# medical-genomics-group/ci-gwas

Measured on AMD Instinct MI355X. Metric: ci_tests_per_sec, higher is better.
Workload: dtype f32; 1 GPU; cusk level sweep, one LD block 10000 SNPs x 20 traits, N=16384, alpha=0.0001, max level 5 (north_star headline); correlation matrix from synthetic .bed (Kendall-npn/Pearson) resident in HBM; n_variables=10020, engine=cusk

## Files before the change

ci-gwas_amd/csrc/cusk_internal.h:

```cpp
#pragma once
#include <hip/hip_runtime.h>

#include <cstdint>
#include <cstdio>
#include <string>
#include <vector>

#include "../../include/cusk_hip.h"

namespace cusk {

constexpr int kML = CUSK_ML;
constexpr int kLevels = CUSK_ML + 2;
constexpr unsigned long long kNone = ~0ull;
constexpr int kNumClasses = 5;
constexpr int kClassCap[kNumClasses] = {39, 63, 127, 191, 1 << 30};
constexpr int kThreads = 256;
constexpr int kTmajMinLevelDefault = 6;
constexpr int kCounterSlots = 512;
constexpr size_t kLdsLimit = 160 * 1024;

struct DevBuf
{
    void *p = nullptr;
    size_t cap = 0;
    hipError_t ensure(size_t bytes)
    {
        if (bytes <= cap) return hipSuccess;
        if (p) (void)hipFree(p);
        p = nullptr;
        cap = 0;
        size_t want = bytes + bytes / 4 + 256;
        hipError_t e = hipMalloc(&p, want);
        if (e == hipSuccess) cap = want;
        return e;
    }
    void release()
    {
        if (p) (void)hipFree(p);
        p = nullptr;
        cap = 0;
    }
    template <typename T>
    T *as() const
    {
        return reinterpret_cast<T *>(p);
    }
};

struct LevelCounters;
struct HostGate;
// ... 40 lines not shown
    void *res_pinned = nullptr;
    size_t res_pinned_cap = 0;
    cusk::DevBuf rv, rpos, sel, wpre;
    long long nrec = 0;
    cusk::LevelCounters *hcnt = nullptr;
    unsigned long long *hslots = nullptr;
    long long *hrec_base = nullptr;
    unsigned long long *hcanon = nullptr;
    int *hflag = nullptr;
    std::vector<unsigned long long> binom_host;
    long long binom_rows = 0;
    cusk::HostGate *hgate = nullptr, *hgate_dev = nullptr;
    int run_seq = 0;
    long long item_cap_cur = 0;
    hipEvent_t ev_main[2] = {nullptr, nullptr};
    hipEvent_t ev_run[2] = {nullptr, nullptr};
    hipEvent_t ev_k0[cusk::kLevels], ev_k1[cusk::kLevels], ev_l0[cusk::kLevels], ev_l1[cusk::kLevels];

    int opt_fast = 1;
    int opt_validate = 0;
    int opt_corr_fp4 = 1;
    int opt_pair = 1;
    int opt_rows = 1;
    int opt_vec = 1;
    int opt_overlap = 1;
    int opt_corr_popcount = 0;
    int opt_corr_mxp_f32 = 0;
    int opt_assume_symmetric = 0;
    long long opt_queue_cap = 4ll << 20;
    int opt_hostprof = 0;
    int opt_tmaj_validate_stride = 1;
    int opt_max_staged_classes = -1;
    int opt_tmaj_min_level = cusk::kTmajMinLevelDefault;
    long long opt_chunk = 2048;
    long long opt_chunk0 = 512;
    long long opt_chunk0_low = 256;
    int opt_vec_threads = 64;
    long long opt_item_cap = 1ll << 20;
    int opt_lookahead = 2;
    int opt_sync2 = 1;
    int opt_l1_threads = 0;
    int opt_l1_lds_row = 1;
    int opt_timing = 1;
    long long opt_sep_ws_budget = 4ll << 30;

    int shard_rank = 0, shard_world = 1;
    int shard_host_staging = 0;
    cusk_exchange_fn shard_fn = nullptr;
    void *shard_user = nullptr;
    void *shard_host = nullptr;
    size_t shard_host_cap = 0;

    cusk::DevBuf bed_dev, phen_dev, mean_dev, std_dev, planes, mxp_dev, pxp_dev, mxp_bq;
    cusk::DevBuf pc_masks, pc_counts;
    cusk::DevBuf corr_tab[2];
    void *corr_tab_pinned[2] = {nullptr, nullptr};
    size_t corr_tab_pinned_cap[2] = {0, 0};
    hipEvent_t ev_corr[5] = {nullptr, nullptr, nullptr, nullptr, nullptr};
    float corr_ms[4] = {0, 0, 0, 0};
};

namespace cusk {

inline int fail(cusk_engine *e, int code, const std::string &msg)
{
    if (e) e->err = msg;
// ... 35 lines not shown
```

ci-gwas_amd/csrc/engine.hip:

```cpp
#include <algorithm>
#include <atomic>
#include <chrono>
#include <cmath>
#include <cstdlib>
#include <cstring>

#include "sweep_common.h"

namespace cusk {

static unsigned long long binom_sat(int n, int k)
{
    if (k < 0 || k > n) return 0;
    if (k > n - k) k = n - k;
    unsigned long long r = 1;
    const unsigned long long cap = 1ull << 62;
    for (int i = 1; i <= k; i++)
    {
        unsigned long long f = (unsigned long long)(n - k + i);
        if (r > cap / f) return cap;
        r = r * f / (unsigned long long)i;
    }
    return r;
}
// ... 22 lines not shown
    const float *C;
    const float *Ness;
    float ess_uniform;
    const int *Ginit;
    const float *Th;
    const int *time_index;
    int n;
    int maxlevel;
    const int2 *row_range = nullptr;
    int max_span = 0;
    long long level0_pairs = 0;
};

constexpr size_t kCtlCnt = 0;
constexpr size_t kCtlSlots = (kCtlCnt + sizeof(LevelCounters) * kLevels + 15) & ~(size_t)15;
constexpr size_t kCtlRecBase = (kCtlSlots + sizeof(unsigned long long) * kLevels * kCounterSlots * 4 + 15) & ~(size_t)15;
constexpr size_t kCtlCanon = (kCtlRecBase + sizeof(long long) * (kLevels + 1) + 15) & ~(size_t)15;
constexpr size_t kCtlSym = (kCtlCanon + sizeof(unsigned long long) * kLevels * kCounterSlots + 15) & ~(size_t)15;
constexpr size_t kCtlBytes = kCtlSym + 16;

struct LevelPlan
{
    SweepParams sp;
    FinalizeParams fp;
    long long nitems[kNumClasses];
    bool use_pair = false, use_fast = false, use_rows = false, filter_ok = true;
    size_t pair_lds = 0;
    bool redone = false;
    bool known_items = false;
    int maxdeg_bound = 0;
    int staged_classes = 0;
    unsigned long long chunk0 = 0;
    bool tmaj = false;
    bool force_exact = false;
};

static int run_levels(cusk_engine *e, const RunArgs &a, cusk_stats *st)
{
    const int n = a.n;
    if (n <= 0 || a.C == nullptr || a.Th == nullptr) return fail(e, CUSK_ERR_ARG, "bad arguments");
    const auto hp_t0 = std::chrono::steady_clock::now();
    std::string hp_log;
    auto hp_mark = [&](const char *what) {
        if (!e->opt_hostprof) return;
        const double us = std::chrono::duration<double, std::micro>(std::chrono::steady_clock::now() - hp_t0).count();
        char buf[64];
        std::snprintf(buf, sizeof(buf), " %s=%.1f", what, us);
        hp_log += buf;
    };
    CUSK_HIP(e, hipSetDevice(e->device));
    hipStream_t s = e->stream;
    const int words = (n + 63) / 64;
    e->n = n;
    e->words = words;
    e->mode = a.mode;
    e->have_result = false;
    e->nrec = 0;
    cusk_stats local;
    std::memset(&local, 0, sizeof(local));
    const bool het = (a.Ness != nullptr);
    const bool het0 = het && a.mode == 0;
    const int last_level = std::min(kML, a.maxlevel);
    const bool sharded = e->shard_world > 1;
    if (sharded && !e->shard_fn) return fail(e, CUSK_ERR_ARG, "row sharding needs an exchange function");

    const size_t bm = sizeof(unsigned long long) * (size_t)n * words;
// ... 101 lines not shown
        }
        const bool fork = (nonempty > 1) && (e->opt_overlap != 0);
        if (fork)
        {
            CUSK_HIP(e, hipEventRecord(e->ev_fork, s));
            CUSK_HIP(e, hipStreamWaitEvent(e->stream2, e->ev_fork, 0));
        }
        bool first = true;
        for (int c = 0; c < kNumClasses; c++)
        {
            if (!may[c]) continue;
            hipStream_t cs = (fork && !first) ? e->stream2 : s;
            first = false;
            sp.items = e->items[l & 1][c].as<int2>();
            sp.cap = kClassCap[c];
            sp.cls = c;
            sp.chunk = (c == 0) ? pl.chunk0 : chunk;
            sp.item_cap = item_cap;
            sp.grid_cap = item_cap;
            if (l >= 2 && !pl.use_pair && !pl.tmaj)
            {
                const int dmax = std::min(pl.maxdeg_bound, kClassCap[c]);
                const unsigned long long sets = binom_sat(dmax, l);
                const unsigned long long per_row = sets / sp.chunk + 1ull;
                if (per_row < (1ull << 40)) sp.grid_cap = std::min<long long>(item_cap, (long long)(per_row * (unsigned long long)n));
            }
            sp.validate = e->opt_validate ? std::max(1, e->opt_tmaj_validate_stride) : 0;
            if (pl.use_pair && !exact_only)
                CUSK_HIP(e, launch_pair(a.mode, sp, pl.pair_lds, cs));
            else if (pl.tmaj && pl.use_fast && !exact_only)
                CUSK_HIP(e, launch_sweep_tmaj(a.mode, l, sp, c, cs));
            else if (pl.use_fast && !exact_only && !het && e->opt_vec && !e->opt_validate && c < kNumClasses - 1 &&
                     sweep_vec_lds_bytes(c) <= kLdsLimit && l < kVecMaxLevel)
                CUSK_HIP(e, launch_sweep_vec(a.mode, l, sp, c, c == 0 ? e->opt_vec_threads : kThreads, cs));
            else if (pl.use_fast && !exact_only)
                CUSK_HIP(e, launch_sweep_fast(a.mode, het, l, e->opt_validate != 0, sp, c, cs));
            else
                CUSK_HIP(e, launch_sweep_exact(a.mode, het, l, sp, c, cs));
        }
        if (fork)
        {
            CUSK_HIP(e, hipEventRecord(e->ev_join, e->stream2));
            CUSK_HIP(e, hipStreamWaitEvent(s, e->ev_join, 0));
        }
        if (pl.use_fast && !exact_only) CUSK_HIP(e, launch_recheck(a.mode, het, l, sp, s));
        return CUSK_OK;
    };
    auto launch_level_finalize = [&](int l) -> int {
        if (a.mode != 0) return CUSK_OK;
        LevelPlan &pl = plan[l];
        pl.fp.qcap = qcap_gate[l];
        CUSK_HIP(e, launch_finalize(l, pl.fp, s));
        return CUSK_OK;
    };

    auto shard_join = [&](int l) -> int {
        LevelPlan &pl = plan[l];
        if (pl.use_fast && l >= 2)
        {
            CUSK_HIP(e, hipMemcpyAsync(e->hcnt + l, dcnt + l, sizeof(LevelCounters), hipMemcpyDeviceToHost, s));
            CUSK_HIP(e, hipStreamSynchronize(s));
            if (e->hcnt[l].qcount > (unsigned long long)e->opt_queue_cap)
            {
                pl.redone = true;
                local.exact_fallbacks++;
                qcap_gate[l] = ~0ull;
                const int rc = launch_level_sweeps(l, true);
// ... 92 lines not shown
                    if (rc != CUSK_OK) return rc;
                    if (!e->hgate[k].active) break;
                }
            }
            if (e->opt_timing == 2) CUSK_HIP(e, hipEventRecord(e->ev_l0[l], s));
            LevelPlan &pl = plan[l];
            pl.redone = false;
            pl.known_items = false;
            const bool first_build = (l == 1 && first_pass);
            int *off_l = (l == 1) ? e->off1.as<int>() : e->off[cs].as<int>();
            PlanArgs pa;
            pa.deg = e->deg.as<int>();
            pa.off = off_l;
            for (int c = 0; c < kNumClasses; c++) pa.items[c] = e->items[cs][c].as<int2>();
            pa.n = n;
            pa.L = l;
            pa.binom = e->binom.as<unsigned long long>();
            pa.chunk = chunk;
            {
                float th_l;
                if (het)
                    th_l = a.Th[0];
                else if (a.mode == 0)
                    th_l = a.Th[l];
                else
                    th_l = uniform_ess_threshold(a.Th[0], a.ess_uniform, l);
                const bool vec0 = (e->opt_fast != 0) && l >= 2 && l < kVecMaxLevel && th_l >= kThMinFilter && !het && e->opt_vec &&
                                  !e->opt_validate && staged_classes > 0;
                const unsigned long long c0 = (l <= 4) ? (unsigned long long)std::max<long long>(e->opt_chunk0_low, 64) : chunk0;
                plan[l].chunk0 = vec0 ? c0 : chunk;
                plan[l].tmaj = (e->opt_fast != 0) && !plan[l].force_exact && l >= std::max(2, e->opt_tmaj_min_level) && l <= kML &&
                               th_l >= kThMinFilter && !het && symmetric && !sharded;
                if (plan[l].tmaj) plan[l].chunk0 = chunk;
            }
            pa.chunk0 = plan[l].chunk0;
            pa.Lsets = plan[l].tmaj ? l + 1 : l;
            pa.staged_classes = staged_classes;
            pa.pair_mode = ((l == 1) && !first_build && plan[l].use_pair && !plan[l].use_rows) ? 1 : 0;
            pa.cnt = dcnt + l;
            pa.prev = (l >= 2) ? dcnt + (l - 1) : nullptr;
            pa.prev_qcap = (l >= 2) ? qcap_gate[l - 1] : ~0ull;
            pa.item_cap = item_cap;
            pa.shard_rank = e->shard_rank;
            pa.shard_world = e->shard_world;
            pa.gate = e->hgate_dev + l;
            pa.seq = run_seq;
            pa.sym = (l == 1 && !e->opt_assume_symmetric && !a.row_range) ? dsym : nullptr;
            pa.blocks = e->planblk.as<unsigned long long>();
            pa.blk_seq = ++e->plan_seq;
            if (first_build && e->binom_rows <= 0)
            {
                CUSK_HIP(e, e->binom.ensure(sizeof(unsigned long long) * kBinomStride));
                pa.binom = e->binom.as<unsigned long long>();
            }
            CUSK_HIP(e, launch_plan(pa, s));
            planned_last = l;
            if (first_build)
            {
                hp_mark("plan1_enq");
                int *const rec_l_before = (a.mode == 0) ? e->rec_l.as<int>() : nullptr;
                const size_t rec_l_cleared = rec_l_before ? e->rec_l.cap : 0;
                if (rec_l_cleared) CUSK_HIP(e, hipMemsetAsync(rec_l_before, 0, rec_l_cleared, s));
                int rc = wait_gate(1);
                if (rc != CUSK_OK) return rc;
                hp_mark("gate1");
                symmetric = (e->hgate[1].sym == 0) || (e->opt_assume_symmetric != 0) || (a.row_range != nullptr);
// ... 71 lines not shown
                maxdeg2 = e->hgate[2].maxdeg;
            }
            {
                pl.maxdeg_bound = maxdeg1;
                if (maxdeg2 >= 0 && l >= 2) pl.maxdeg_bound = std::min(pl.maxdeg_bound, maxdeg2);
                const int k = l - 1 - lookahead;
                if (k >= 1 && e->hgate[k].seq == run_seq && e->hgate[k].active) pl.maxdeg_bound = std::min(pl.maxdeg_bound, e->hgate[k].maxdeg);
                pl.staged_classes = staged_classes;
            }

            SweepParams &sp = pl.sp;
            sp.C = a.C;
            sp.Ness = a.Ness;
            sp.n = n;
            sp.level = l;
            sp.off = off_l;
            sp.nbr = e->nbr[cs].as<int>();
            sp.best = e->best[cs].as<unsigned long long>();
            sp.adj = e->adj.as<unsigned long long>();
            sp.deg = e->deg.as<int>();
            sp.words = words;
            sp.items = nullptr;
            sp.binom = e->binom.as<unsigned long long>();
            sp.time_index = e->ti.as<int>();
            sp.has_ti = (a.mode == 1 && a.time_index != nullptr) ? 1 : 0;
            sp.chunk = chunk;
            sp.cap = 0;
            sp.cls = 0;
            sp.item_cap = item_cap;
            sp.grid_cap = item_cap;
            sp.cnt = dcnt + l;
            sp.row_range = a.row_range;
            sp.max_span = a.row_range ? a.max_span : n;
            sp.slots = dslots + (size_t)l * kCounterSlots * 4;
            if (het)
                sp.th = a.Th[0];
            else if (a.mode == 0)
                sp.th = a.Th[l];
            else
                sp.th = uniform_ess_threshold(a.Th[0], a.ess_uniform, l);
            {
                const double tq = std::tanh((double)sp.th);
                sp.t2 = (float)(tq * tq);
                pl.filter_ok = (sp.th >= kThMinFilter);
                if (!pl.filter_ok) pl.use_fast = false;
            }
            sp.queue = nullptr;
            sp.qcap = 0;
            qcap_gate[l] = ~0ull;
            if (pl.use_fast)
            {
                sp.queue = e->queue.as<RecheckEntry>();
                sp.qcap = (unsigned long long)e->opt_queue_cap;
                qcap_gate[l] = sp.qcap;
            }
            FinalizeParams &fp = pl.fp;
            fp.C = a.C;
            fp.n = n;
            fp.off = sp.off;
            fp.nbr = sp.nbr;
            fp.best = sp.best;
            fp.sel = pl.use_rows ? e->sel.as<unsigned>() : nullptr;
            fp.level = l;
            fp.adj = sp.adj;
            fp.deg = sp.deg;
            fp.words = words;
// ... 274 lines not shown
{
    if (!e || !key) return CUSK_ERR_ARG;
    const std::string k(key);
    if (k == "fast")
        e->opt_fast = (int)value;
    else if (k == "validate")
        e->opt_validate = (int)value;
    else if (k == "corr_fp4")
        e->opt_corr_fp4 = (int)value;
    else if (k == "pair")
        e->opt_pair = (int)value;
    else if (k == "rows")
        e->opt_rows = (int)value;
    else if (k == "vec")
        e->opt_vec = (int)value;
    else if (k == "overlap")
        e->opt_overlap = (int)value;
    else if (k == "corr_popcount")
        e->opt_corr_popcount = (int)value;
    else if (k == "corr_mxp_f32")
        e->opt_corr_mxp_f32 = (int)value;
    else if (k == "assume_symmetric")
        e->opt_assume_symmetric = (int)value;
    else if (k == "queue_capacity" && value > 0)
        e->opt_queue_cap = value;
    else if (k == "chunk" && value >= 256)
        e->opt_chunk = value;
    else if (k == "max_staged_classes")
        e->opt_max_staged_classes = (int)value;
    else if (k == "tmaj_validate_stride" && value >= 1 && (value & (value - 1)) == 0)
        e->opt_tmaj_validate_stride = (int)value;
    else if (k == "tmaj_min_level")
        e->opt_tmaj_min_level = (int)value;
    else if (k == "hostprof")
        e->opt_hostprof = (int)value;
    else if (k == "chunk0_low" && value >= 64)
        e->opt_chunk0_low = value;
    else if (k == "chunk0" && value >= 64)
        e->opt_chunk0 = value;
    else if (k == "vec_threads" && (value == 64 || value == 128 || value == 256))
        e->opt_vec_threads = (int)value;
    else if (k == "item_capacity" && value > 0)
    {
        e->opt_item_cap = value;
        e->item_cap_cur = 0;
    }
    else if (k == "lookahead" && value >= 0)
        e->opt_lookahead = (int)value;
    else if (k == "timing")
        e->opt_timing = (int)value;
    else if (k == "l1_threads" && (value == 0 || value == 256 || value == 512))
        e->opt_l1_threads = (int)value;
    else if (k == "l1_lds_row" && (value == 0 || value == 1))
        e->opt_l1_lds_row = (int)value;
    else if (k == "sync2")
        e->opt_sync2 = (int)value;
    else if (k == "sepselect_ws_bytes" && value > 0)
        e->opt_sep_ws_budget = value;
    else
        return fail(e, CUSK_ERR_ARG, "unknown option " + k);
    return CUSK_OK;
}

extern "C" int cusk_engine_set_row_shard(cusk_engine *e, int rank, int world, cusk_exchange_fn fn, void *user, int host_staging)
{
    if (!e) return CUSK_ERR_ARG;
// ... 514 lines not shown
```

ci-gwas_amd/csrc/sweep_common.h:

```cpp
#pragma once
#include "cusk_internal.h"

namespace cusk {

constexpr int kBinomStride = 16;
constexpr int kVecMaxLevel = 9;
constexpr float kThMinFilter = 2e-3f;

struct RowInfo
{
    int cls;
    int base;
    int nchunks;
    int pad;
};

struct RecheckEntry
{
    int x;
    int k2;
    unsigned long long rank;
};

struct LevelCounters
// ... 19 lines not shown
    long long class_items[kNumClasses];
};

struct SweepParams
{
    const float *C;
    const float *Ness;
    int n;
    int level;
    const int *off;
    const int *nbr;
    unsigned long long *best;
    unsigned long long *adj;
    int *deg;
    int words;
    const int2 *items;
    const unsigned long long *binom;
    const int *time_index;
    int has_ti;
    float th;
    float t2;
    unsigned long long chunk;
    int cap;
    int cls;
    long long item_cap;
    long long grid_cap;
    LevelCounters *cnt;
    unsigned long long *slots;
    RecheckEntry *queue;
    unsigned long long qcap;
    int validate;
    const int2 *row_range;
    int max_span;
};

struct FinalizeParams
{
    const float *C;
    int n;
    const int *off;
    const int *nbr;
    const unsigned long long *best;
    const unsigned *sel;
    int level;
    unsigned long long *adj;
    int *deg;
    int words;
    const unsigned long long *binom;
    const int *off1;
    const int *wpre1;
    const unsigned long long *adj0;
    int *rec_x, *rec_y, *rec_l, *rec_s;
    long long rec_cap;
    const int4 *meta;
    const LevelCounters *cnt;
    unsigned long long qcap;
    unsigned long long *slots;
    unsigned long long *canon;
};

__host__ __device__ inline size_t align16(size_t x) { return (x + 15) & ~(size_t)15; }

struct LdsLayout
{
    size_t nbr, best, ti, sub, ess, total;
};
// ... 82 lines not shown
}

__device__ __forceinline__ bool clear_edge(unsigned long long *adj, int *deg, int words, int X, int Y)
{
    const unsigned long long o1 = atomicAnd(&adj[(size_t)X * words + (Y >> 6)], ~(1ull << (Y & 63)));
    const unsigned long long o2 = atomicAnd(&adj[(size_t)Y * words + (X >> 6)], ~(1ull << (X & 63)));
    const bool f1 = (o1 >> (Y & 63)) & 1ull, f2 = (o2 >> (X & 63)) & 1ull;
    if (f1) atomicSub(&deg[X], 1);
    if (f2) atomicSub(&deg[Y], 1);
    return f1;
}
#endif

hipError_t launch_sweep_exact(int mode, bool het, int L, const SweepParams &p, int cls, hipStream_t st);
hipError_t launch_recheck(int mode, bool het, int L, const SweepParams &p, hipStream_t st);
hipError_t launch_finalize(int L, const FinalizeParams &p, hipStream_t st);
hipError_t launch_record_z(int L, const float *C, int n, const int *x, const int *y, const int *l, const int *s, long long stride,
                           long long count, float *z, hipStream_t st);
constexpr int kRecBlock = 1024;
hipError_t launch_rec_count(const int *rec_l, long long slots, int *counts, hipStream_t st);
hipError_t launch_rec_compact(const int *rec_l, const int *rec_x, const int *rec_y, const int *rec_s, long long rec_cap,
                              long long slots, const long long *block_off, int *out_x, int *out_y, int *out_l, int *out_s,
                              long long out_stride, hipStream_t st);
hipError_t launch_sweep_fast(int mode, bool het, int L, bool validate, const SweepParams &p, int cls, hipStream_t st);
hipError_t launch_sweep_tmaj(int mode, int L, const SweepParams &p, int cls, hipStream_t st);
__host__ __device__ inline int tmaj_prefixes_per_lane(int d, int s, unsigned long long chunk)
{
    const unsigned long long r = (unsigned long long)(d - 1 - s);
    const unsigned long long pairs = r * (r - 1ull) / 2ull;
    const unsigned long long k = chunk / ((unsigned long long)kThreads * (pairs ? pairs : 1ull));
    return (int)(k < 1ull ? 1ull : (k > 64ull ? 64ull : k));
}
hipError_t launch_sweep_vec(int mode, int L, const SweepParams &p, int cls, int threads, hipStream_t st);
unsigned persistent_grid(const void *kernel, int threads, size_t lds);
size_t sweep_vec_lds_bytes(int cls);
hipError_t launch_level0(const float *C, const float *Ness, const int *Ginit, unsigned long long *adj, int n, int words,
                         float th, int *asym_flag, hipStream_t st);
hipError_t launch_level0_batch(const float *C, const float *Ness, unsigned long long *adj, unsigned long long *adj0, int *deg, int n,
                               int words, const int2 *row_range, float th, hipStream_t st);
hipError_t launch_degree(const unsigned long long *adj, int *deg, int n, int words, unsigned long long *adj0, hipStream_t st);
hipError_t launch_fill_nbr(const unsigned long long *adj, const int *off, int *nbr, unsigned long long *best, int n, int words,
                           int *wpre, const LevelCounters *cnt, const int2 *row_range, hipStream_t st);
struct PlanArgs
{
    const int *deg;
    int *off;
    int2 *items[kNumClasses];
    int n, L;
    int Lsets;
    const unsigned long long *binom;
    unsigned long long chunk, chunk0;
    int staged_classes, pair_mode;
    LevelCounters *cnt;
    const LevelCounters *prev;
    unsigned long long prev_qcap;
    long long item_cap;
    int shard_rank, shard_world;
    HostGate *gate;
    int seq;
    const int *sym;
    unsigned long long *blocks;
    unsigned blk_seq;
};
hipError_t launch_plan(const PlanArgs &a, hipStream_t st);
hipError_t launch_expand_records(const int *rec_s, const int *rec_l, long long rec_cap, long long count, int *out,
                                 hipStream_t st);
// ... 18 lines not shown
```

ci-gwas_amd/csrc/sweep_vec.hip:

```cpp
#include <algorithm>

#include "ci_fast.h"
#include "sweep_common.h"

namespace cusk {

typedef float f2 __attribute__((ext_vector_type(2)));
typedef float f4 __attribute__((ext_vector_type(4)));
typedef unsigned int u4 __attribute__((ext_vector_type(4)));

__host__ __device__ inline int vec_ld4(int d)
{
    int ld = (d + 1 + 3) & ~3;
    if ((ld & 7) == 0) ld += 4;
    return ld;
}

struct VecLayout
{
    size_t rel, rowx, nbr, ti, sub, bin, total;
};
constexpr int kVecBinCols = kVecMaxLevel - 2;
__host__ __device__ inline VecLayout vec_layout(int cap)
{
    VecLayout l;
    const size_t dp = (size_t)((cap + 4) & ~3);
    l.rel = 0;
    l.rowx = align16(l.rel + sizeof(unsigned) * dp);
    l.nbr = align16(l.rowx + sizeof(float) * dp);
    l.ti = align16(l.nbr + sizeof(int) * (cap + 1));
    l.sub = align16(l.ti + sizeof(int) * (cap + 1));
    l.bin = align16(l.sub + sizeof(float) * (size_t)(cap + 1) * vec_ld4(cap));
    l.total = align16(l.bin + sizeof(unsigned long long) * (size_t)kVecBinCols * (cap + 1));
    return l;
}

template <int L>
__device__ __forceinline__ void unrank_comb_lds(unsigned long long rem, int d, const unsigned long long *s_bin, int ldb, int *idx)
{
    int c = 0;
#pragma unroll
    for (int i = 0; i < L; i++)
    {
        if (i == L - 1)
        {
            idx[i] = c + (int)rem;
            break;
        }
        const unsigned long long *col = s_bin + (L - 2 - i) * ldb;
        while (true)
        {
            const unsigned long long b = col[d - 1 - c];
            if (rem < b) break;
            rem -= b;
            c++;
        }
        idx[i] = c;
        c++;
    }
}

template <int L, int MODE, int THREADS>
__global__ void __launch_bounds__(THREADS) sweep_vec_kernel(SweepParams p)
{
    static_assert(L >= 2, "level 1 has its own kernels");
    extern __shared__ __attribute__((aligned(16))) unsigned char smem[];
    __shared__ unsigned long long s_cnt[4];

    const int n = p.n;
    const int tid = threadIdx.x;
    const VecLayout lay = vec_layout(p.cap);
    unsigned *s_rel = reinterpret_cast<unsigned *>(smem + lay.rel);
    float *s_rowx = reinterpret_cast<float *>(smem + lay.rowx);
    int *s_nbr = reinterpret_cast<int *>(smem + lay.nbr);
    int *s_ti = reinterpret_cast<int *>(smem + lay.ti);
    float *s_sub = reinterpret_cast<float *>(smem + lay.sub);
    unsigned long long *s_bin = reinterpret_cast<unsigned long long *>(smem + lay.bin);
    const int ldb = p.cap + 1;
    if (tid < 4) s_cnt[tid] = 0ull;
    for (int e = tid; e < (L - 1) * ldb; e += THREADS)
    {
        const int b = e / ldb, a = e - b * ldb;
        s_bin[e] = p.binom[(size_t)a * kBinomStride + (b + 1)];
    }
    unsigned long long ntests = 0, nsub = 0, nrem = 0;
    const long long nitems = level_items(p);
    int2 item_next = ((long long)blockIdx.x < nitems) ? p.items[blockIdx.x] : make_int2(0, 0);
    for (long long it = blockIdx.x; it < nitems; it += gridDim.x)
    {
    if (it != (long long)blockIdx.x) __syncthreads();
    const int2 item = item_next;
    if (it + gridDim.x < nitems) item_next = p.items[it + gridDim.x];
    const int X = item.x;
    const int o0 = p.off[X];
    const int d = p.off[X + 1] - o0;
    const int ld4 = vec_ld4(d);
    const int dp = (d + 3) & ~3;
    const int *g_nbr = p.nbr + o0;

    const unsigned long long ncomb = p.binom[(size_t)d * kBinomStride + L];
    const unsigned long long r0 = (unsigned long long)item.y * p.chunk;
    const unsigned long long cntr = min(p.chunk, ncomb - r0);

    for (int k = tid; k <= d; k += THREADS)
    {
        const int v = (k < d) ? g_nbr[k] : X;
        s_nbr[k] = v;
        if constexpr (MODE == 1) s_ti[k] = p.time_index[v];
    }
    for (int k = tid; k < dp; k += THREADS)
    {
        unsigned rel = 0u;
        float rx = 0.0f;
        if (k < d)
        {
            const int y = g_nbr[k];
            rx = p.C[(size_t)X * n + y];
            if constexpr (MODE == 0)
            {
                const unsigned long long b = p.best[o0 + k];
                rel = (b == kNone) ? 0xffffffffu : ((b < r0) ? 0u : (unsigned)min(b - r0 + 1ull, 0xfffffffeull));
            }
            else
            {
                const unsigned long long wv = p.adj[(size_t)X * p.words + (y >> 6)];
                rel = ((wv >> (y & 63)) & 1ull) ? 0xffffffffu : 0u;
            }
        }
        s_rel[k] = rel;
        s_rowx[k] = rx;
    }
    {
        constexpr int kU = 8;
        const int total = d * dp;
        const int di = THREADS % dp, dj = THREADS / dp;
        int j = tid / dp, i = tid - j * dp;
        for (int e0 = tid; e0 < total; e0 += THREADS * kU)
        {
            float v[kU];
            int at[kU];
#pragma unroll
            for (int u = 0; u < kU; u++)
            {
                const bool in = (e0 + u * THREADS < total);
                at[u] = in ? j * ld4 + i : -1;
                const float c = p.C[(size_t)g_nbr[min(i, d - 1)] * n + g_nbr[min(j, d - 1)]];
                v[u] = (i < d) ? c : 0.0f;
                i += di;
                j += dj;
                if (i >= dp)
                {
                    i -= dp;
                    j++;
                }
            }
#pragma unroll
            for (int u = 0; u < kU; u++)
                if (at[u] >= 0) s_sub[at[u]] = v[u];
        }
    }
    __syncthreads();

    const unsigned long long q = (cntr + THREADS - 1) / THREADS;
    const unsigned long long lo = r0 + (unsigned long long)tid * q;
// ... 8 lines not shown
        for (unsigned long long rank = lo; rank < hi; rank++)
        {
            const unsigned myrel = (unsigned)(rank - r0) + 1u;
            SubsetFast<L> fx;
            {
                float cl[SubsetFast<L>::NL], m1x[L];
#pragma unroll
                for (int a = 0; a < L; a++) m1x[a] = s_rowx[idx[a]];
#pragma unroll
                for (int a = 1; a < L; a++)
#pragma unroll
                    for (int b = 0; b < a; b++) cl[a * (a - 1) / 2 + b] = s_sub[idx[a] * ld4 + idx[b]];
                fx.prepare(cl, m1x);
            }
            nsub++;
            [[maybe_unused]] int tmaxS = 0;
            if constexpr (MODE == 1)
            {
                tmaxS = s_ti[idx[0]];
#pragma unroll
                for (int a = 1; a < L; a++) tmaxS = max(tmaxS, s_ti[idx[a]]);
            }
            const float *col[L];
#pragma unroll
            for (int a = 0; a < L; a++) col[a] = s_sub + idx[a] * ld4;
            const f2 h00v = {fx.h00, fx.h00};
            bool anyalive = false;
            [[maybe_unused]] unsigned long long smask = 0ull;
            if constexpr (THREADS == 64)
            {
#pragma unroll
                for (int a = 0; a < L; a++) smask |= 1ull << idx[a];
            }
            for (int g = 0; g < dp; g += 4)
            {
                const u4 rel = *reinterpret_cast<const u4 *>(s_rel + g);
                unsigned livem = (rel.x >= myrel ? 1u : 0u) | (rel.y >= myrel ? 2u : 0u) | (rel.z >= myrel ? 4u : 0u) |
                                 (rel.w >= myrel ? 8u : 0u);
                anyalive |= (livem != 0u);
                if constexpr (THREADS == 64)
                    livem &= ~((unsigned)(smask >> g) & 15u);
                else
                {
#pragma unroll
                    for (int a = 0; a < L; a++)
                        if ((idx[a] >> 2) == (g >> 2)) livem &= ~(1u << (idx[a] & 3));
                }
                if constexpr (MODE == 1)
                {
                    if (p.has_ti)
                    {
#pragma unroll
                        for (int u = 0; u < 4; u++)
                            if (tmaxS > max(tiX, s_ti[min(g + u, d)])) livem &= ~(1u << u);
                    }
                }
                if (livem == 0u) continue;
                f4 my[L];
#pragma unroll
                for (int a = 0; a < L; a++) my[a] = *reinterpret_cast<const f4 *>(col[a] + g);
                const f4 m0 = *reinterpret_cast<const f4 *>(s_rowx + g);
                f2 bA[L], bB[L];
                f2 h11A = {1.0f, 1.0f}, h11B = {1.0f, 1.0f};
                f2 h01A = {m0.x, m0.y}, h01B = {m0.z, m0.w};
#pragma unroll
                for (int i = 0; i < L; i++)
                {
                    f2 sA = {my[i].x, my[i].y}, sB = {my[i].z, my[i].w};
#pragma unroll
                    for (int k = 0; k < i; k++)
                    {
                        const float fik = fx.f[i * (i - 1) / 2 + k];
                        const f2 nf = {-fik, -fik};
                        sA = __builtin_elementwise_fma(nf, bA[k], sA);
                        sB = __builtin_elementwise_fma(nf, bB[k], sB);
                    }
                    const f2 iv = {fx.invd[i], fx.invd[i]};
                    bA[i] = sA * iv;
                    bB[i] = sB * iv;
                    h11A = __builtin_elementwise_fma(-bA[i], bA[i], h11A);
                    h11B = __builtin_elementwise_fma(-bB[i], bB[i], h11B);
                    const f2 na = {-fx.a[i], -fx.a[i]};
                    h01A = __builtin_elementwise_fma(na, bA[i], h01A);
                    h01B = __builtin_elementwise_fma(na, bB[i], h01B);
                }
                const f2 prodA = h00v * h11A, prodB = h00v * h11B;
                const f2 lhsA = h01A * h01A, lhsB = h01B * h01B;
                const f2 loA = prodA * t2lo, loB = prodB * t2lo, hiA = prodA * t2hi, hiB = prodB * t2hi;
                ntests += __popc(livem);
                unsigned failq;
                {
                    const f2 dA = lhsA - hiA, dB = lhsB - hiB;
                    const f2 eA = h11A - kCondMin, eB = h11B - kCondMin;
                    failq = ((dA.x > 0.0f && eA.x > 0.0f) ? 1u : 0u) | ((dA.y > 0.0f && eA.y > 0.0f) ? 2u : 0u) |
                            ((dB.x > 0.0f && eB.x > 0.0f) ? 4u : 0u) | ((dB.y > 0.0f && eB.y > 0.0f) ? 8u : 0u);
                }
                if (!fx.ill && (livem & ~failq) == 0u) continue;
                unsigned passm = 0u, failm = 0u;
                passm |= (h11A.x >= kCondMin && lhsA.x < loA.x) ? 1u : 0u;
                passm |= (h11A.y >= kCondMin && lhsA.y < loA.y) ? 2u : 0u;
                passm |= (h11B.x >= kCondMin && lhsB.x < loB.x) ? 4u : 0u;
                passm |= (h11B.y >= kCondMin && lhsB.y < loB.y) ? 8u : 0u;
                failm |= (h11A.x >= kCondMin && lhsA.x > hiA.x) ? 1u : 0u;
                failm |= (h11A.y >= kCondMin && lhsA.y > hiA.y) ? 2u : 0u;
                failm |= (h11B.x >= kCondMin && lhsB.x > hiB.x) ? 4u : 0u;
                failm |= (h11B.y >= kCondMin && lhsB.y > hiB.y) ? 8u : 0u;
                if (fx.ill)
                {
                    passm = 0u;
                    failm = 0u;
                }
                unsigned todo = livem & ~failm;
                while (todo)
                {
                    const int u = __ffs(todo) - 1;
                    todo &= todo - 1;
                    const int k2 = g + u;
                    if ((passm >> u) & 1u)
                    {
                        bool first;
                        if constexpr (MODE == 0)
                        {
                            const unsigned long long old = atomicMin(&p.best[o0 + k2], rank);
                            atomicMin(&s_rel[k2], myrel);
                            first = (old == kNone);
                        }
                        else
                        {
                            first = clear_edge(p.adj, p.deg, p.words, X, s_nbr[k2]);
                            s_rel[k2] = 0u;
                        }
                        if (first) nrem++;
                    }
                    else
                    {
                        const unsigned long long qi = atomicAdd(&p.cnt->qcount, 1ull);
                        if (qi < p.qcap)
                        {
                            RecheckEntry en;
                            en.x = X;
                            en.k2 = k2;
                            en.rank = rank;
                            p.queue[qi] = en;
                        }
                    }
                }
            }
            if (!anyalive) break;
            {
                int i = L - 1;
                while (i >= 0 && idx[i] == d - L + i) i--;
                if (i < 0) break;
                idx[i]++;
                for (int j2 = i + 1; j2 < L; j2++) idx[j2] = idx[j2 - 1] + 1;
            }
        }
    }
    }
    for (int o = 32; o > 0; o >>= 1)
    {
        ntests += __shfl_xor(ntests, o);
        nsub += __shfl_xor(nsub, o);
        nrem += __shfl_xor(nrem, o);
    }
    __syncthreads();
    if ((tid & 63) == 0)
    {
        if (ntests) atomicAdd(&s_cnt[0], ntests);
        if (nsub) atomicAdd(&s_cnt[1], nsub);
        if (MODE == 1 && nrem) atomicAdd(&s_cnt[2], nrem);
    }
    __syncthreads();
    if (tid == 0)
    {
        unsigned long long *sl = p.slots + (size_t)(blockIdx.x & (kCounterSlots - 1)) * 4;
        for (int i = 0; i < 3; i++)
            if (s_cnt[i]) atomicAdd(&sl[i], s_cnt[i]);
    }
}
// ... 49 lines not shown
```

Before: 247.3 billion CI tests/s.

## Add prefix-sharing sweep kernel for small-degree class at levels 4-5

```diff
diff --git a/ci-gwas_amd/csrc/cusk_internal.h b/ci-gwas_amd/csrc/cusk_internal.h
--- a/ci-gwas_amd/csrc/cusk_internal.h
+++ b/ci-gwas_amd/csrc/cusk_internal.h
@@ -17,6 +17,7 @@
 constexpr int kClassCap[kNumClasses] = {39, 63, 127, 191, 1 << 30};
 constexpr int kThreads = 256;
 constexpr int kTmajMinLevelDefault = 6;
+constexpr int kPrefixMinLevelDefault = 4;
 constexpr int kCounterSlots = 512;
 constexpr size_t kLdsLimit = 160 * 1024;
 
@@ -123,6 +124,7 @@
     int opt_tmaj_validate_stride = 1;
     int opt_max_staged_classes = -1;
     int opt_tmaj_min_level = cusk::kTmajMinLevelDefault;
+    int opt_prefix_min_level = cusk::kPrefixMinLevelDefault;
     long long opt_chunk = 2048;
     long long opt_chunk0 = 512;
     long long opt_chunk0_low = 256;
diff --git a/ci-gwas_amd/csrc/engine.hip b/ci-gwas_amd/csrc/engine.hip
--- a/ci-gwas_amd/csrc/engine.hip
+++ b/ci-gwas_amd/csrc/engine.hip
@@ -78,6 +78,7 @@
     int staged_classes = 0;
     unsigned long long chunk0 = 0;
     bool tmaj = false;
+    bool prefix = false;
     bool force_exact = false;
 };
 
@@ -245,7 +246,12 @@
                 CUSK_HIP(e, launch_sweep_tmaj(a.mode, l, sp, c, cs));
             else if (pl.use_fast && !exact_only && !het && e->opt_vec && !e->opt_validate && c < kNumClasses - 1 &&
                      sweep_vec_lds_bytes(c) <= kLdsLimit && l < kVecMaxLevel)
-                CUSK_HIP(e, launch_sweep_vec(a.mode, l, sp, c, c == 0 ? e->opt_vec_threads : kThreads, cs));
+            {
+                if (c == 0 && pl.prefix)
+                    CUSK_HIP(e, launch_sweep_prefix(l, sp, c, cs));
+                else
+                    CUSK_HIP(e, launch_sweep_vec(a.mode, l, sp, c, c == 0 ? e->opt_vec_threads : kThreads, cs));
+            }
             else if (pl.use_fast && !exact_only)
                 CUSK_HIP(e, launch_sweep_fast(a.mode, het, l, e->opt_validate != 0, sp, c, cs));
             else
@@ -404,6 +410,8 @@
                 plan[l].tmaj = (e->opt_fast != 0) && !plan[l].force_exact && l >= std::max(2, e->opt_tmaj_min_level) && l <= kML &&
                                th_l >= kThMinFilter && !het && symmetric && !sharded;
                 if (plan[l].tmaj) plan[l].chunk0 = chunk;
+                plan[l].prefix = vec0 && !plan[l].tmaj && a.mode == 0 && symmetric && l >= std::max(3, e->opt_prefix_min_level) &&
+                                 l <= kPrefixMaxLevel;
             }
             pa.chunk0 = plan[l].chunk0;
             pa.Lsets = plan[l].tmaj ? l + 1 : l;
@@ -881,6 +889,8 @@
         e->opt_tmaj_validate_stride = (int)value;
     else if (k == "tmaj_min_level")
         e->opt_tmaj_min_level = (int)value;
+    else if (k == "prefix_min_level")
+        e->opt_prefix_min_level = (int)value;
     else if (k == "hostprof")
         e->opt_hostprof = (int)value;
     else if (k == "chunk0_low" && value >= 64)
diff --git a/ci-gwas_amd/csrc/sweep_common.h b/ci-gwas_amd/csrc/sweep_common.h
--- a/ci-gwas_amd/csrc/sweep_common.h
+++ b/ci-gwas_amd/csrc/sweep_common.h
@@ -223,6 +223,8 @@
     return (int)(k < 1ull ? 1ull : (k > 64ull ? 64ull : k));
 }
 hipError_t launch_sweep_vec(int mode, int L, const SweepParams &p, int cls, int threads, hipStream_t st);
+constexpr int kPrefixMaxLevel = 5;
+hipError_t launch_sweep_prefix(int L, const SweepParams &p, int cls, hipStream_t st);
 unsigned persistent_grid(const void *kernel, int threads, size_t lds);
 size_t sweep_vec_lds_bytes(int cls);
 hipError_t launch_level0(const float *C, const float *Ness, const int *Ginit, unsigned long long *adj, int n, int words,
diff --git a/ci-gwas_amd/csrc/sweep_prefix.hip b/ci-gwas_amd/csrc/sweep_prefix.hip
--- /dev/null
+++ b/ci-gwas_amd/csrc/sweep_prefix.hip
@@ -0,0 +1,361 @@
+#include <algorithm>
+
+#include "ci_fast.h"
+#include "sweep_common.h"
+#include "sweep_stage.h"
+#include "sweep_vec_layout.h"
+
+namespace cusk {
+
+constexpr int kPreStride = 40;
+constexpr int kPreBatch = 6;
+static_assert(((kClassCap[0] + 3) & ~3) <= kPreStride, "component rows hold the first degree class");
+
+struct PrefixLayout
+{
+    size_t pre, hdr, set, total;
+};
+__host__ __device__ inline PrefixLayout prefix_layout(int cap, int L)
+{
+    PrefixLayout l;
+    l.pre = vec_layout(cap).total;
+    l.hdr = align16(l.pre + sizeof(float) * (size_t)kPreBatch * (L + 1) * kPreStride);
+    l.set = align16(l.hdr + sizeof(float) * kPreBatch);
+    l.total = align16(l.set + sizeof(uint2) * (size_t)kPreBatch * kPreStride);
+    return l;
+}
+
+template <int L, int THREADS = 64>
+__global__ void __launch_bounds__(THREADS) sweep_prefix_kernel(SweepParams p)
+{
+    static_assert(L >= 3 && L < kVecMaxLevel, "levels 3 and up (a prefix of at least two members)");
+    static_assert(THREADS == 64, "one wavefront per work item");
+    constexpr int LP = L - 1;
+    constexpr int PS = (L + 1) * kPreStride;
+    extern __shared__ __attribute__((aligned(16))) unsigned char smem[];
+
+    const int n = p.n;
+    const int tid = threadIdx.x;
+    const VecLayout lay = vec_layout(p.cap);
+    const PrefixLayout play = prefix_layout(p.cap, L);
+    unsigned *s_rel = reinterpret_cast<unsigned *>(smem + lay.rel);
+    float *s_rowx = reinterpret_cast<float *>(smem + lay.rowx);
+    float *s_sub = reinterpret_cast<float *>(smem + lay.sub);
+    unsigned long long *s_bin = reinterpret_cast<unsigned long long *>(smem + lay.bin);
+    float *s_pre = reinterpret_cast<float *>(smem + play.pre);
+    float *s_hdr = reinterpret_cast<float *>(smem + play.hdr);
+    uint2 *s_set = reinterpret_cast<uint2 *>(smem + play.set);
+    const int ldb = p.cap + 1;
+    for (int e = tid; e < (L - 1) * ldb; e += THREADS)
+    {
+        const int b = e / ldb, a = e - b * ldb;
+        s_bin[e] = p.binom[(size_t)a * kBinomStride + (b + 1)];
+    }
+    unsigned long long ntests_all = 0, nsub = 0;
+    const float t2lo = p.t2 * (1.0f - kBeta), t2hi = p.t2 * (1.0f + kBeta);
+    const long long nitems = level_items(p);
+    int2 item_next = ((long long)blockIdx.x < nitems) ? p.items[blockIdx.x] : make_int2(0, 0);
+    for (long long it = blockIdx.x; it < nitems; it += gridDim.x)
+    {
+    __syncthreads();
+    const int2 item = item_next;
+    if (it + gridDim.x < nitems) item_next = p.items[it + gridDim.x];
+    const int X = item.x;
+    const int o0 = p.off[X];
+    const int d = p.off[X + 1] - o0;
+    const int ld4 = vec_ld4(d);
+    const int dp = (d + 3) & ~3;
+    const int *g_nbr = p.nbr + o0;
+
+    const unsigned long long ncomb = p.binom[(size_t)d * kBinomStride + L];
+    const unsigned long long r0 = (unsigned long long)item.y * p.chunk;
+    const unsigned rend = (unsigned)min(p.chunk, ncomb - r0);
+
+    for (int k = tid; k < dp; k += THREADS)
+    {
+        unsigned rel = 0u;
+        float rx = 0.0f;
+        if (k < d)
+        {
+            rx = p.C[(size_t)X * n + g_nbr[k]];
+            const unsigned long long b = p.best[o0 + k];
+            rel = (b == kNone) ? 0xffffffffu : ((b < r0) ? 0u : (unsigned)min(b - r0 + 1ull, 0xfffffffeull));
+        }
+        s_rel[k] = rel;
+        s_rowx[k] = rx;
+    }
+    {
+        constexpr int kU = 8;
+        const int total = d * dp;
+        const int di = THREADS % dp, dj = THREADS / dp;
+        int j = tid / dp, i = tid - j * dp;
+        for (int e0 = tid; e0 < total; e0 += THREADS * kU)
+        {
+            float v[kU];
+            int at[kU];
+#pragma unroll
+            for (int u = 0; u < kU; u++)
+            {
+                const bool in = (e0 + u * THREADS < total);
+                at[u] = in ? j * ld4 + i : -1;
+                const float c = p.C[(size_t)g_nbr[min(i, d - 1)] * n + g_nbr[min(j, d - 1)]];
+                v[u] = (i < d) ? c : 0.0f;
+                i += di;
+                j += dj;
+                if (i >= dp)
+                {
+                    i -= dp;
+                    j++;
+                }
+            }
+#pragma unroll
+            for (int u = 0; u < kU; u++)
+                if (at[u] >= 0) s_sub[at[u]] = v[u];
+        }
+    }
+    __syncthreads();
+
+    const int NG = dp >> 2;
+    const unsigned magic = 65536u / (unsigned)NG + 1u;
+    const int npb_max = min(THREADS / NG, kPreBatch);
+    const int a_pi = (int)(__umul24((unsigned)tid, magic) >> 16);
+    const int a_g = (tid - a_pi * NG) * 4;
+
+    int P[LP], sfirst;
+    {
+        int idx[L];
+        unrank_comb_lds<L>(r0, d, s_bin, ldb, idx);
+#pragma unroll
+        for (int a = 0; a < LP; a++) P[a] = __builtin_amdgcn_readfirstlane(idx[a]);
+        sfirst = __builtin_amdgcn_readfirstlane(idx[L - 1]);
+    }
+    unsigned rr = 0u;
+    unsigned ntests = 0u;
+    while (rr < rend)
+    {
+        const unsigned rr0 = rr;
+        unsigned myP = 0u;
+        int nsets = 0, npb = 0;
+        for (int pi = 0; pi < npb_max && rr < rend; pi++)
+        {
+            const int ns = (int)min((unsigned)(d - sfirst), rend - rr);
+            unsigned packed = 0u;
+            unsigned long long pm = 0ull;
+#pragma unroll
+            for (int a = 0; a < LP; a++)
+            {
+                packed |= (unsigned)P[a] << (8 * a);
+                pm |= 1ull << P[a];
+            }
+            if (a_pi == pi) myP = packed;
+            if (tid < ns)
+            {
+                const int s = sfirst + tid;
+                const unsigned long long sm = pm | (1ull << s);
+                s_set[nsets + tid] = make_uint2((unsigned)s | ((unsigned)pi << 8) | ((unsigned)(sm >> 32) << 16), (unsigned)sm);
+            }
+            nsets += ns;
+            rr += (unsigned)ns;
+            npb = pi + 1;
+            next_comb_pos<LP>(P, d - 1);
+            sfirst = P[LP - 1] + 1;
+        }
+
+        if (nsets <= 0) break;
+
+        if (a_pi < npb)
+        {
+            int Pi[LP];
+#pragma unroll
+            for (int a = 0; a < LP; a++) Pi[a] = (int)((myP >> (8 * a)) & 255u);
+            SubsetFast<LP> fx;
+            {
+                float cl[SubsetFast<LP>::NL], m1x[LP];
+#pragma unroll
+                for (int a = 0; a < LP; a++) m1x[a] = s_rowx[Pi[a]];
+#pragma unroll
+                for (int a = 1; a < LP; a++)
+#pragma unroll
+                    for (int b = 0; b < a; b++) cl[a * (a - 1) / 2 + b] = s_sub[Pi[a] * ld4 + Pi[b]];
+                fx.prepare(cl, m1x);
+            }
+            f4 my[LP];
+#pragma unroll
+            for (int a = 0; a < LP; a++) my[a] = *reinterpret_cast<const f4 *>(s_sub + Pi[a] * ld4 + a_g);
+            const f4 m0 = *reinterpret_cast<const f4 *>(s_rowx + a_g);
+            f2 bA[LP], bB[LP];
+            f2 h11A = {1.0f, 1.0f}, h11B = {1.0f, 1.0f};
+            f2 h01A = {m0.x, m0.y}, h01B = {m0.z, m0.w};
+            float *dst = s_pre + a_pi * PS + a_g;
+#pragma unroll
+            for (int i = 0; i < LP; i++)
+            {
+                f2 sA = {my[i].x, my[i].y}, sB = {my[i].z, my[i].w};
+#pragma unroll
+                for (int k = 0; k < i; k++)
+                {
+                    const float fik = fx.f[i * (i - 1) / 2 + k];
+                    const f2 nf = {-fik, -fik};
+                    sA = __builtin_elementwise_fma(nf, bA[k], sA);
+                    sB = __builtin_elementwise_fma(nf, bB[k], sB);
+                }
+                const f2 iv = {fx.invd[i], fx.invd[i]};
+                bA[i] = sA * iv;
+                bB[i] = sB * iv;
+                h11A = __builtin_elementwise_fma(-bA[i], bA[i], h11A);
+                h11B = __builtin_elementwise_fma(-bB[i], bB[i], h11B);
+                const f2 na = {-fx.a[i], -fx.a[i]};
+                h01A = __builtin_elementwise_fma(na, bA[i], h01A);
+                h01B = __builtin_elementwise_fma(na, bB[i], h01B);
+                const f4 ui = {bA[i].x, bA[i].y, bB[i].x, bB[i].y};
+                *reinterpret_cast<f4 *>(dst + i * kPreStride) = ui;
+            }
+            const f4 ev = {h11A.x, h11A.y, h11B.x, h11B.y}, gv = {h01A.x, h01A.y, h01B.x, h01B.y};
+            *reinterpret_cast<f4 *>(dst + LP * kPreStride) = ev;
+            *reinterpret_cast<f4 *>(dst + L * kPreStride) = gv;
+            if (a_g == 0) s_hdr[a_pi] = fx.ill ? __uint_as_float(0x7fc00000u) : fx.h00;
+        }
+        __syncthreads();
+
+        const unsigned total = (unsigned)(nsets * NG);
+        nsub += (unsigned)nsets;
+        unsigned alive = 0u;
+        unsigned qn = min(__umul24((unsigned)tid, magic) >> 16, (unsigned)(nsets - 1));
+        uint2 swn = s_set[qn];
+        for (unsigned t = (unsigned)tid; t < total; t += THREADS)
+        {
+            const unsigned q = qn;
+            const uint2 sw = swn;
+            qn = min(__umul24(t + THREADS, magic) >> 16, (unsigned)(nsets - 1));
+            swn = s_set[qn];
+            const int g = (int)(t - __umul24(q, (unsigned)NG)) * 4;
+            const int pi = (int)((sw.x >> 8) & 255u), s = (int)(sw.x & 255u);
+            const unsigned myrel = rr0 + q + 1u;
+            const u4 rel = *reinterpret_cast<const u4 *>(s_rel + g);
+            unsigned livem = (rel.x >= myrel ? 1u : 0u) | (rel.y >= myrel ? 2u : 0u) | (rel.z >= myrel ? 4u : 0u) |
+                             (rel.w >= myrel ? 8u : 0u);
+            alive |= livem;
+            const unsigned long long smask = (unsigned long long)sw.y | ((unsigned long long)(sw.x >> 16) << 32);
+            livem &= ~((unsigned)(smask >> g) & 15u);
+            if (livem == 0u) continue;
+
+            const float *ps = s_pre + __umul24((unsigned)pi, (unsigned)PS);
+            float us[LP];
+#pragma unroll
+            for (int k = 0; k < LP; k++) us[k] = ps[k * kPreStride + s];
+            const float es = ps[LP * kPreStride + s], gs = ps[L * kPreStride + s];
+            const float invd = __frsqrt_rn(es);
+            const float aL = gs * invd;
+            const float h00 = __builtin_fmaf(-aL, aL, s_hdr[pi]);
+            const bool ill = !(es >= kCondMin) || !(h00 >= kCondMin);
+            const f4 cy = *reinterpret_cast<const f4 *>(s_sub + __umul24((unsigned)s, (unsigned)ld4) + g);
+            f2 sA = {cy.x, cy.y}, sB = {cy.z, cy.w};
+#pragma unroll
+            for (int k = 0; k < LP; k++)
+            {
+                const f4 uy = *reinterpret_cast<const f4 *>(ps + k * kPreStride + g);
+                const f2 nf = {-us[k], -us[k]};
+                const f2 uA = {uy.x, uy.y}, uB = {uy.z, uy.w};
+                sA = __builtin_elementwise_fma(nf, uA, sA);
+                sB = __builtin_elementwise_fma(nf, uB, sB);
+            }
+            const f2 iv = {invd, invd};
+            const f2 bA = sA * iv, bB = sB * iv;
+            const f4 ey = *reinterpret_cast<const f4 *>(ps + LP * kPreStride + g);
+            const f4 gy4 = *reinterpret_cast<const f4 *>(ps + L * kPreStride + g);
+            const f2 eA = {ey.x, ey.y}, eB = {ey.z, ey.w}, gA = {gy4.x, gy4.y}, gB = {gy4.z, gy4.w};
+            const f2 h11A = __builtin_elementwise_fma(-bA, bA, eA), h11B = __builtin_elementwise_fma(-bB, bB, eB);
+            const f2 na = {-aL, -aL};
+            const f2 h01A = __builtin_elementwise_fma(na, bA, gA), h01B = __builtin_elementwise_fma(na, bB, gB);
+
+            const f2 h00v = {h00, h00};
+            const f2 prodA = h00v * h11A, prodB = h00v * h11B;
+            const f2 lhsA = h01A * h01A, lhsB = h01B * h01B;
+            const f2 loA = prodA * t2lo, loB = prodB * t2lo, hiA = prodA * t2hi, hiB = prodB * t2hi;
+            ntests += __popc(livem);
+            unsigned failq;
+            {
+                const f2 dA = lhsA - hiA, dB = lhsB - hiB;
+                const f2 cA = h11A - kCondMin, cB = h11B - kCondMin;
+                failq = ((dA.x > 0.0f && cA.x > 0.0f) ? 1u : 0u) | ((dA.y > 0.0f && cA.y > 0.0f) ? 2u : 0u) |
+                        ((dB.x > 0.0f && cB.x > 0.0f) ? 4u : 0u) | ((dB.y > 0.0f && cB.y > 0.0f) ? 8u : 0u);
+            }
+            if (!ill && (livem & ~failq) == 0u) continue;
+            unsigned passm = 0u, failm = 0u;
+            passm |= (h11A.x >= kCondMin && lhsA.x < loA.x) ? 1u : 0u;
+            passm |= (h11A.y >= kCondMin && lhsA.y < loA.y) ? 2u : 0u;
+            passm |= (h11B.x >= kCondMin && lhsB.x < loB.x) ? 4u : 0u;
+            passm |= (h11B.y >= kCondMin && lhsB.y < loB.y) ? 8u : 0u;
+            failm |= (h11A.x >= kCondMin && lhsA.x > hiA.x) ? 1u : 0u;
+            failm |= (h11A.y >= kCondMin && lhsA.y > hiA.y) ? 2u : 0u;
+            failm |= (h11B.x >= kCondMin && lhsB.x > hiB.x) ? 4u : 0u;
+            failm |= (h11B.y >= kCondMin && lhsB.y > hiB.y) ? 8u : 0u;
+            if (ill)
+            {
+                passm = 0u;
+                failm = 0u;
+            }
+            const unsigned long long rank = r0 + (unsigned long long)(rr0 + q);
+            unsigned todo = livem & ~failm;
+            while (todo)
+            {
+                const int u = __ffs(todo) - 1;
+                todo &= todo - 1;
+                const int k2 = g + u;
+                if ((passm >> u) & 1u)
+                {
+                    atomicMin(&p.best[o0 + k2], rank);
+                    atomicMin(&s_rel[k2], myrel);
+                }
+                else
+                {
+                    const unsigned long long qi = atomicAdd(&p.cnt->qcount, 1ull);
+                    if (qi < p.qcap)
+                    {
+                        RecheckEntry en;
+                        en.x = X;
+                        en.k2 = k2;
+                        en.rank = rank;
+                        p.queue[qi] = en;
+                    }
+                }
+            }
+        }
+        if (__ballot(alive != 0u) == 0ull) break;
+        __syncthreads();
+    }
+    ntests_all += ntests;
+    }
+    for (int o = 32; o > 0; o >>= 1) ntests_all += __shfl_xor(ntests_all, o);
+    if (tid == 0)
+    {
+        unsigned long long *sl = p.slots + (size_t)(blockIdx.x & (kCounterSlots - 1)) * 4;
+        if (ntests_all) atomicAdd(&sl[0], ntests_all);
+        if (nsub) atomicAdd(&sl[1], nsub);
+    }
+}
+
+template <int L>
+static hipError_t launch_prefix_L(const SweepParams &p, int cls, hipStream_t st)
+{
+    const size_t lds = prefix_layout(kClassCap[cls], L).total;
+    auto kfn = sweep_prefix_kernel<L, 64>;
+    const unsigned grid = (unsigned)std::min<long long>(persistent_grid(reinterpret_cast<const void *>(kfn), 64, lds),
+                                                        std::max<long long>(p.grid_cap, 1));
+    hipLaunchKernelGGL(kfn, dim3(grid), dim3(64), lds, st, p);
+    return hipGetLastError();
+}
+
+hipError_t launch_sweep_prefix(int L, const SweepParams &p, int cls, hipStream_t st)
+{
+    if (cls != 0) return hipErrorInvalidValue;
+    switch (L)
+    {
+    case 3: return launch_prefix_L<3>(p, cls, st);
+    case 4: return launch_prefix_L<4>(p, cls, st);
+    case 5: return launch_prefix_L<5>(p, cls, st);
+    }
+    return hipErrorInvalidValue;
+}
+
+}
diff --git a/ci-gwas_amd/csrc/sweep_vec.hip b/ci-gwas_amd/csrc/sweep_vec.hip
--- a/ci-gwas_amd/csrc/sweep_vec.hip
+++ b/ci-gwas_amd/csrc/sweep_vec.hip
@@ -2,63 +2,9 @@
 
 #include "ci_fast.h"
 #include "sweep_common.h"
+#include "sweep_vec_layout.h"
 
 namespace cusk {
-
-typedef float f2 __attribute__((ext_vector_type(2)));
-typedef float f4 __attribute__((ext_vector_type(4)));
-typedef unsigned int u4 __attribute__((ext_vector_type(4)));
-
-__host__ __device__ inline int vec_ld4(int d)
-{
-    int ld = (d + 1 + 3) & ~3;
-    if ((ld & 7) == 0) ld += 4;
-    return ld;
-}
-
-struct VecLayout
-{
-    size_t rel, rowx, nbr, ti, sub, bin, total;
-};
-constexpr int kVecBinCols = kVecMaxLevel - 2;
-__host__ __device__ inline VecLayout vec_layout(int cap)
-{
-    VecLayout l;
-    const size_t dp = (size_t)((cap + 4) & ~3);
-    l.rel = 0;
-    l.rowx = align16(l.rel + sizeof(unsigned) * dp);
-    l.nbr = align16(l.rowx + sizeof(float) * dp);
-    l.ti = align16(l.nbr + sizeof(int) * (cap + 1));
-    l.sub = align16(l.ti + sizeof(int) * (cap + 1));
-    l.bin = align16(l.sub + sizeof(float) * (size_t)(cap + 1) * vec_ld4(cap));
-    l.total = align16(l.bin + sizeof(unsigned long long) * (size_t)kVecBinCols * (cap + 1));
-    return l;
-}
-
-template <int L>
-__device__ __forceinline__ void unrank_comb_lds(unsigned long long rem, int d, const unsigned long long *s_bin, int ldb, int *idx)
-{
-    int c = 0;
-#pragma unroll
-    for (int i = 0; i < L; i++)
-    {
-        if (i == L - 1)
-        {
-            idx[i] = c + (int)rem;
-            break;
-        }
-        const unsigned long long *col = s_bin + (L - 2 - i) * ldb;
-        while (true)
-        {
-            const unsigned long long b = col[d - 1 - c];
-            if (rem < b) break;
-            rem -= b;
-            c++;
-        }
-        idx[i] = c;
-        c++;
-    }
-}
 
 template <int L, int MODE, int THREADS>
 __global__ void __launch_bounds__(THREADS) sweep_vec_kernel(SweepParams p)
diff --git a/ci-gwas_amd/csrc/sweep_vec_layout.h b/ci-gwas_amd/csrc/sweep_vec_layout.h
--- /dev/null
+++ b/ci-gwas_amd/csrc/sweep_vec_layout.h
@@ -0,0 +1,61 @@
+#pragma once
+#include "sweep_common.h"
+
+namespace cusk {
+
+typedef float f2 __attribute__((ext_vector_type(2)));
+typedef float f4 __attribute__((ext_vector_type(4)));
+typedef unsigned int u4 __attribute__((ext_vector_type(4)));
+
+__host__ __device__ inline int vec_ld4(int d)
+{
+    int ld = (d + 1 + 3) & ~3;
+    if ((ld & 7) == 0) ld += 4;
+    return ld;
+}
+
+struct VecLayout
+{
+    size_t rel, rowx, nbr, ti, sub, bin, total;
+};
+constexpr int kVecBinCols = kVecMaxLevel - 2;
+__host__ __device__ inline VecLayout vec_layout(int cap)
+{
+    VecLayout l;
+    const size_t dp = (size_t)((cap + 4) & ~3);
+    l.rel = 0;
+    l.rowx = align16(l.rel + sizeof(unsigned) * dp);
+    l.nbr = align16(l.rowx + sizeof(float) * dp);
+    l.ti = align16(l.nbr + sizeof(int) * (cap + 1));
+    l.sub = align16(l.ti + sizeof(int) * (cap + 1));
+    l.bin = align16(l.sub + sizeof(float) * (size_t)(cap + 1) * vec_ld4(cap));
+    l.total = align16(l.bin + sizeof(unsigned long long) * (size_t)kVecBinCols * (cap + 1));
+    return l;
+}
+
+template <int L>
+__device__ __forceinline__ void unrank_comb_lds(unsigned long long rem, int d, const unsigned long long *s_bin, int ldb, int *idx)
+{
+    int c = 0;
+#pragma unroll
+    for (int i = 0; i < L; i++)
+    {
+        if (i == L - 1)
+        {
+            idx[i] = c + (int)rem;
+            break;
+        }
+        const unsigned long long *col = s_bin + (L - 2 - i) * ldb;
+        while (true)
+        {
+            const unsigned long long b = col[d - 1 - c];
+            if (rem < b) break;
+            rem -= b;
+            c++;
+        }
+        idx[i] = c;
+        c++;
+    }
+}
+
+}
```

After: 188.2 billion CI tests/s. -23.9%, worse.

## Use wave bitmasks for live-neighbor checks and load symmetric submatrix half

Applied to the files above, without the earlier changes.

```diff
diff --git a/ci-gwas_amd/csrc/engine.hip b/ci-gwas_amd/csrc/engine.hip
--- a/ci-gwas_amd/csrc/engine.hip
+++ b/ci-gwas_amd/csrc/engine.hip
@@ -541,6 +541,7 @@
             sp.cnt = dcnt + l;
             sp.row_range = a.row_range;
             sp.max_span = a.row_range ? a.max_span : n;
+            sp.symmetric = symmetric ? 1 : 0;
             sp.slots = dslots + (size_t)l * kCounterSlots * 4;
             if (het)
                 sp.th = a.Th[0];
diff --git a/ci-gwas_amd/csrc/sweep_common.h b/ci-gwas_amd/csrc/sweep_common.h
--- a/ci-gwas_amd/csrc/sweep_common.h
+++ b/ci-gwas_amd/csrc/sweep_common.h
@@ -75,6 +75,7 @@
     int validate;
     const int2 *row_range;
     int max_span;
+    int symmetric;
 };
 
 struct FinalizeParams
diff --git a/ci-gwas_amd/csrc/sweep_vec.hip b/ci-gwas_amd/csrc/sweep_vec.hip
--- a/ci-gwas_amd/csrc/sweep_vec.hip
+++ b/ci-gwas_amd/csrc/sweep_vec.hip
@@ -66,6 +66,7 @@
     static_assert(L >= 2, "level 1 has its own kernels");
     extern __shared__ __attribute__((aligned(16))) unsigned char smem[];
     __shared__ unsigned long long s_cnt[4];
+    __shared__ __attribute__((aligned(16))) unsigned long long s_mask[2];
 
     const int n = p.n;
     const int tid = threadIdx.x;
@@ -108,6 +109,7 @@
         s_nbr[k] = v;
         if constexpr (MODE == 1) s_ti[k] = p.time_index[v];
     }
+    [[maybe_unused]] unsigned rel_mine = 0u;
     for (int k = tid; k < dp; k += THREADS)
     {
         unsigned rel = 0u;
@@ -129,7 +131,59 @@
         }
         s_rel[k] = rel;
         s_rowx[k] = rx;
-    }
+        rel_mine = rel;
+    }
+    if constexpr (THREADS == 64 && MODE == 0)
+    {
+        const unsigned long long la = __ballot(rel_mine == 0xffffffffu);
+        const unsigned long long mx = __ballot(rel_mine != 0u && rel_mine != 0xffffffffu);
+        if (tid == 0)
+        {
+            s_mask[0] = la;
+            s_mask[1] = mx;
+        }
+    }
+    if (p.symmetric)
+    {
+        constexpr int kU = 8;
+        const int W = d + 1;
+        const int total = ((d + 1) >> 1) * W;
+        const int dc = THREADS % W, dr = THREADS / W;
+        int r = tid / W, c = tid - r * W;
+        for (int e0 = tid; e0 < total; e0 += THREADS * kU)
+        {
+            float v[kU];
+            int at[kU], at2[kU];
+#pragma unroll
+            for (int u = 0; u < kU; u++)
+            {
+                const bool in = (e0 + u * THREADS < total);
+                const bool first = (c <= r);
+                const int j = first ? r : d - 1 - r;
+                const int i = first ? c : c - r - 1;
+                at[u] = in ? j * ld4 + i : -1;
+                at2[u] = i * ld4 + j;
+                v[u] = p.C[(size_t)g_nbr[min(max(i, 0), d - 1)] * n + g_nbr[min(max(j, 0), d - 1)]];
+                c += dc;
+                r += dr;
+                if (c >= W)
+                {
+                    c -= W;
+                    r++;
+                }
+            }
+#pragma unroll
+            for (int u = 0; u < kU; u++)
+                if (at[u] >= 0)
+                {
+                    s_sub[at[u]] = v[u];
+                    s_sub[at2[u]] = v[u];
+                }
+        }
+        for (int j = tid; j < d; j += THREADS)
+            for (int i = d; i < dp; i++) s_sub[j * ld4 + i] = 0.0f;
+    }
+    else
     {
         constexpr int kU = 8;
         const int total = d * dp;
@@ -204,20 +258,7 @@
 #pragma unroll
                 for (int a = 0; a < L; a++) smask |= 1ull << idx[a];
             }
-            for (int g = 0; g < dp; g += 4)
-            {
-                const u4 rel = *reinterpret_cast<const u4 *>(s_rel + g);
-                unsigned livem = (rel.x >= myrel ? 1u : 0u) | (rel.y >= myrel ? 2u : 0u) | (rel.z >= myrel ? 4u : 0u) |
-                                 (rel.w >= myrel ? 8u : 0u);
-                anyalive |= (livem != 0u);
-                if constexpr (THREADS == 64)
-                    livem &= ~((unsigned)(smask >> g) & 15u);
-                else
-                {
-#pragma unroll
-                    for (int a = 0; a < L; a++)
-                        if ((idx[a] >> 2) == (g >> 2)) livem &= ~(1u << (idx[a] & 3));
-                }
+            auto group = [&](const int g, unsigned livem) __attribute__((always_inline)) {
                 if constexpr (MODE == 1)
                 {
                     if (p.has_ti)
@@ -227,7 +268,7 @@
                             if (tmaxS > max(tiX, s_ti[min(g + u, d)])) livem &= ~(1u << u);
                     }
                 }
-                if (livem == 0u) continue;
+                if (livem == 0u) return;
                 f4 my[L];
 #pragma unroll
                 for (int a = 0; a < L; a++) my[a] = *reinterpret_cast<const f4 *>(col[a] + g);
@@ -267,7 +308,7 @@
                     failq = ((dA.x > 0.0f && eA.x > 0.0f) ? 1u : 0u) | ((dA.y > 0.0f && eA.y > 0.0f) ? 2u : 0u) |
                             ((dB.x > 0.0f && eB.x > 0.0f) ? 4u : 0u) | ((dB.y > 0.0f && eB.y > 0.0f) ? 8u : 0u);
                 }
-                if (!fx.ill && (livem & ~failq) == 0u) continue;
+                if (!fx.ill && (livem & ~failq) == 0u) return;
                 unsigned passm = 0u, failm = 0u;
                 passm |= (h11A.x >= kCondMin && lhsA.x < loA.x) ? 1u : 0u;
                 passm |= (h11A.y >= kCondMin && lhsA.y < loA.y) ? 2u : 0u;
@@ -295,6 +336,11 @@
                         {
                             const unsigned long long old = atomicMin(&p.best[o0 + k2], rank);
                             atomicMin(&s_rel[k2], myrel);
+                            if constexpr (THREADS == 64)
+                            {
+                                atomicOr(&s_mask[1], 1ull << k2);
+                                atomicAnd(&s_mask[0], ~(1ull << k2));
+                            }
                             first = (old == kNone);
                         }
                         else
@@ -317,6 +363,37 @@
                         }
                     }
                 }
+            };
+            bool bymask = false;
+            if constexpr (THREADS == 64 && MODE == 0)
+            {
+                const unsigned long long live_all = s_mask[0], mixed = s_mask[1];
+                if (mixed == 0ull)
+                {
+                    bymask = true;
+                    anyalive = (live_all != 0ull);
+                    const unsigned long long cand = live_all & ~smask;
+                    for (int g = 0; g < dp; g += 4) group(g, (unsigned)(cand >> g) & 15u);
+                }
+            }
+            if (!bymask)
+            {
+                for (int g = 0; g < dp; g += 4)
+                {
+                    const u4 rel = *reinterpret_cast<const u4 *>(s_rel + g);
+                    unsigned livem = (rel.x >= myrel ? 1u : 0u) | (rel.y >= myrel ? 2u : 0u) | (rel.z >= myrel ? 4u : 0u) |
+                                     (rel.w >= myrel ? 8u : 0u);
+                    anyalive |= (livem != 0u);
+                    if constexpr (THREADS == 64)
+                        livem &= ~((unsigned)(smask >> g) & 15u);
+                    else
+                    {
+#pragma unroll
+                        for (int a = 0; a < L; a++)
+                            if ((idx[a] >> 2) == (g >> 2)) livem &= ~(1u << (idx[a] & 3));
+                    }
+                    group(g, livem);
+                }
             }
             if (!anyalive) break;
             {
```

New measurement: 251.4 billion CI tests/s before, 256.1 billion CI tests/s after (median of 6 runs). 1.9% higher.
